# addam/mesh-reconstruction

Hardware: AMD Instinct MI355X
Metric: cost-volume samples/sec (pixels x planes x views) (higher is better)
Workload: dtype u8

## Files before the change

mesh-reconstruction_amd/csrc/sweep_rect.hip:

```cpp
#include "sweep_shared.hpp"

#include <cstddef>
#include <cstdio>
#include <cstdlib>
#include <cstring>
#include <type_traits>
#include <vector>

namespace mvs {

namespace {

constexpr float RX_MAGIC = 12582912.0f;
constexpr int RX_TILE_H = 8, RX_PC = 16, RX_KW = 4;
constexpr int RX_MAX_NI = 3;
#ifndef RX_DOUBLE_BUFFER
#define RX_DOUBLE_BUFFER 0
#endif
#ifndef RX_WAVES
#define RX_WAVES 5
#endif
constexpr int RX_WAVES_PER_SIMD = RX_WAVES;

enum RxMode : unsigned { RX_SKIP = 0, RX_FAST = 1, RX_BORDER = 2, RX_GENERIC = 3 };
// ... 247 lines not shown
    const RectCold *__restrict__ cold;
    uint2 *__restrict__ part;
    size_t pad_slab;
    int pitch, W, H, D, V, v0, vcount, nchunks, chunk0, chunk1, cps, ty0, tyn, tiles_x;
    int slot_dw;
};

template <typename T>
__device__ __forceinline__ T cold_get(uintptr_t c, size_t off)
{
    return *(const __attribute__((address_space(4))) T *)(c + off);
}
#define RX_COLD(c, T, field) cold_get<T>((uintptr_t)(c), offsetof(RectCold, field))

__device__ __forceinline__ __amdgpu_buffer_rsrc_t make_rsrc(const void *p, uint32_t bytes)
{
    return __builtin_amdgcn_make_buffer_rsrc((void *)p, 0, (int)bytes, 0x00020000);
}

template <int RS, bool WRITE_VOLUME, bool FUSED>
__global__ __launch_bounds__(256, RX_WAVES_PER_SIMD) void sweep_fx_rect(RectArgs a)
{
    constexpr int UNITS = RS / 4;
    constexpr int SLOT_BIAS_DW = RX_BIAS_X + RX_BIAS_Y * RS;
    extern __shared__ __attribute__((aligned(16))) uint32_t smem[];
    const uint32_t lds_base = (uint32_t)(size_t)(__attribute__((address_space(3))) void *)smem;

    const int band_tile = grouped_tile(blockIdx.x, a.tiles_x, a.tyn);
    if (band_tile < 0) return;
    const int tx = band_tile % a.tiles_x, ty = band_tile / a.tiles_x + a.ty0;
    const int lane = threadIdx.x & 63;
    const int wave = __builtin_amdgcn_readfirstlane((int)(threadIdx.x >> 6));
    const int col = tx * TILE_W + lane;
    const int row0 = ty * RX_TILE_H;
    const bool col_ok = col < a.W;
    const int NC = a.nchunks;

    uint32_t Im255[8];
    {
        const uint8_t *img = RX_COLD(a.cold, const uint8_t *, main_img);
#pragma unroll
        for (int j = 0; j < 8; j++) Im255[j] = (col_ok && row0 + j < a.H) ? 255u * (uint32_t)img[(size_t)(row0 + j) * a.W + col] : 0u;
    }

    uint32_t srcoff[RX_MAX_NI];
#pragma unroll
    for (int t = 0; t < RX_MAX_NI; t++) {
        const int g = (wave + 4 * t) * 64 + lane;
        srcoff[t] = 4u * (uint32_t)((g / UNITS) * a.pitch + (g % UNITS) * 4);
    }

    const int chunk_first = a.chunk0 + (int)blockIdx.y * a.cps;
    const int chunk_last = min(a.chunk1, chunk_first + a.cps);
    const int vend = a.v0 + a.vcount;
    const int nreg = (chunk_last - chunk_first) * a.vcount;

    const __amdgpu_buffer_rsrc_t rtab = make_rsrc(a.xw, 0xffffffffu);
    const uint32_t xw_wg = (uint32_t)(((size_t)tx * a.V * NC * 4 + wave) * 32);
    const uint32_t yr_wg = (uint32_t)((size_t)((const char *)a.yr - (const char *)a.xw) + ((size_t)ty * a.V * NC * 4 + wave) * 32);
    const __amdgpu_buffer_rsrc_t rquads = make_rsrc(a.quads, 0xffffffffu);

    auto issue_copy = [&](uint32_t xsx, uint32_t ysrc, uint32_t yn, uint32_t slot_dw0) {
        const int n = (int)((yn & 0xffu) * (xsx >> 16));
        const uint32_t src = (xsx & 0xffffu) + ysrc;
        uint32_t *dst = smem + slot_dw0 + SLOT_BIAS_DW + wave * 256;
        const int left = n - wave * 64;
        auto copy = [&](int t, bool whole) {
            int lim = left - 256 * t;
            asm volatile("" : "+s"(lim));
            if (whole || lane < lim)
                __builtin_amdgcn_raw_ptr_buffer_load_lds(rquads, (__attribute__((address_space(3))) void *)(dst + t * 1024), 16, srcoff[t], src, 0, 0);
        };
        static_assert(RX_MAX_NI == 3, "the nest below");
        if (left >= 64) {
            copy(0, true);
            if (left >= 320) {
                copy(1, true);
                if (left >= 576)
                    copy(2, true);
                else if (left > 512)
                    copy(2, false);
            } else if (left > 256) {
                copy(1, false);
            }
        } else if (left > 0) {
            copy(0, false);
        }
    };

    const uint32_t lane8 = 4u * (uint32_t)(lane & 7);
    auto load_x = [&](uint32_t xo) { return __builtin_amdgcn_raw_buffer_load_b32(rtab, lane8, xo, 0); };
    auto load_y = [&](uint32_t yo) { return __builtin_amdgcn_raw_buffer_load_b32(rtab, lane8, yo, 0); };
    auto rdl = [](uint32_t x, int l) { return (uint32_t)__builtin_amdgcn_readlane((int)x, l); };
    struct Cursor {
        int vleft, left;
        uint32_t xo;
    };
    const uint32_t xstep = 128u * (uint32_t)NC;
    const int vlast = a.vcount - 1;
    const uint32_t xwrap = 128u - xstep * (uint32_t)vlast;
    auto advance = [&](Cursor &c) {
        if (c.left <= 0) return;
        c.left--;
        const bool wrap = c.vleft == 0;
        c.xo += wrap ? xwrap : xstep;
        c.vleft = wrap ? vlast : c.vleft - 1;
    };
    const uint32_t x_first = xw_wg + 128u * (uint32_t)(a.v0 * NC + chunk_first);
    const uint32_t ydelta = yr_wg - xw_wg;

    uint32_t acc[8][RX_KW];
    uint32_t best[8];
    int bi[8];
#pragma unroll
    for (int j = 0; j < 8; j++) {
        best[j] = 0xffffffffu;
        bi[j] = -1;
#pragma unroll
        for (int k = 0; k < RX_KW; k++) acc[j][k] = 0u;
    }
    bool plain = true;
    uint32_t spacc = 0u;

    Cursor c2;
    c2.vleft = vlast;
    c2.left = nreg - 1;
    c2.xo = x_first;
    uint32_t x0r = load_x(c2.xo), y0r = load_y(c2.xo + ydelta);
    advance(c2);
    uint32_t x1r = load_x(c2.xo), y1r = load_y(c2.xo + ydelta);
    advance(c2);
    uint32_t slot_cur = 0u, slot_nxt = (uint32_t)a.slot_dw;
    if (nreg > 0) issue_copy(rdl(x0r, 6), rdl(y0r, 2), rdl(y0r, 3), slot_cur);
    int chunk = chunk_first, v = a.v0;

    for (int r = 0; r < nreg; r++) {
        wait_vm<0>();
        __builtin_amdgcn_s_barrier();
        if (r + 1 < nreg) issue_copy(rdl(x1r, 6), rdl(y1r, 2), rdl(y1r, 3), slot_nxt);
        const uint32_t x2r = load_x(c2.xo), y2r = load_y(c2.xo + ydelta);
        advance(c2);
        const uint32_t rsum = x0r + y0r;
        const uint32_t sum01 = rdl(rsum, 0), sum23 = rdl(rsum, 1);
        const uint32_t we[RX_KW] = {rdl(x0r, 2), rdl(x0r, 3), rdl(x0r, 4), rdl(x0r, 5)};
        const uint32_t fmask = 0xffffu;
        const uint32_t fld[RX_KW] = {sum01 & fmask, (sum01 >> 16) & fmask, sum23 & fmask, (sum23 >> 16) & fmask};

        const uint32_t special = (sum01 | sum23) & 0xc000c000u;
        {
            const uint32_t slot_byte = lds_base + slot_cur * 4u;
            uint32_t qd[1][8];
            const uint32_t xmasks = rdl(x0r, 7), ymasks = rdl(y0r, 4);
            const uint32_t anymask = xmasks | ymasks;
            if (__builtin_expect(anymask != 0u, 0)) {
#pragma unroll
                for (int k = 0; k < RX_KW; k++)
                    if (((anymask >> (8 * k)) & 0xffu) && !(fld[k] & 0xc000u)) spacc += 1u << (8 * k);
            }
#define RX_ROW_TAIL(j)                                                                                                   \
    "s_bitcmp0_b32 %[ym], %[yb" #j "]\n\ts_cselect_b64 exec, vcc, 0\n\tv_add_u32 %[a" #j "], 0x1000000, %[a" #j "]\n\t" \
    "v_sad_u16 %[a" #j "], %[q" #j "], %[i" #j "], %[a" #j "]\n\t"
#pragma unroll
            for (int k = 0; k < RX_KW; k++) {
#pragma clang diagnostic push
#pragma clang diagnostic ignored "-Winline-asm"
                asm volatile("s_add_u32 m0, %[slot], %[fld]\n\t"
                             "s_and_b32 vcc_lo, %[fld], 0xc000\n\t"
                             "ds_read_addtid_b32 %[q0] offset:%[o0]\n\tds_read_addtid_b32 %[q1] offset:%[o1]\n\tds_read_addtid_b32 %[q2] offset:%[o2]\n\tds_read_addtid_b32 %[q3] offset:%[o3]\n\t"
                             "ds_read_addtid_b32 %[q4] offset:%[o4]\n\tds_read_addtid_b32 %[q5] offset:%[o5]\n\tds_read_addtid_b32 %[q6] offset:%[o6]\n\tds_read_addtid_b32 %[q7] offset:%[o7]\n\t"
                             "s_cselect_b64 exec, 0, -1\n\t"
                             "s_bfe_u32 vcc_lo, %[am], %[kb]\n\t"
                             "s_cbranch_scc1 1f\n\t"
                             "s_waitcnt lgkmcnt(0)\n\t"
                             "v_dot4_u32_u8 %[q0], %[q0], %[w], 0\n\tv_dot4_u32_u8 %[q1], %[q1], %[w], 0\n\tv_dot4_u32_u8 %[q2], %[q2], %[w], 0\n\tv_dot4_u32_u8 %[q3], %[q3], %[w], 0\n\t"
                             "v_dot4_u32_u8 %[q4], %[q4], %[w], 0\n\tv_dot4_u32_u8 %[q5], %[q5], %[w], 0\n\tv_dot4_u32_u8 %[q6], %[q6], %[w], 0\n\tv_dot4_u32_u8 %[q7], %[q7], %[w], 0\n\t"
                             "v_sad_u16 %[a0], %[q0], %[i0], %[a0]\n\tv_sad_u16 %[a1], %[q1], %[i1], %[a1]\n\tv_sad_u16 %[a2], %[q2], %[i2], %[a2]\n\tv_sad_u16 %[a3], %[q3], %[i3], %[a3]\n\t"
                             "v_sad_u16 %[a4], %[q4], %[i4], %[a4]\n\tv_sad_u16 %[a5], %[q5], %[i5], %[a5]\n\tv_sad_u16 %[a6], %[q6], %[i6], %[a6]\n\tv_sad_u16 %[a7], %[q7], %[i7], %[a7]\n\t"
                             "2:\n\t"
                             "s_mov_b64 exec, -1\n\t"
                             "s_branch 9f\n\t"
                             "1:\n\t"
                             "s_bfe_u32 vcc_lo, %[xm], %[nb]\n\t"
                             "s_bitcmp1_b32 %[xm], %[sb]\n\t"
                             "s_cbranch_scc1 3f\n\t"
                             "s_lshl_b64 exec, exec, vcc_lo\n\t"
                             "s_branch 4f\n\t"
                             "3:\n\t"
                             "s_lshr_b64 exec, exec, vcc_lo\n\t"
                             "4:\n\t"
                             "s_bitcmp1_b32 %[xm], %[eb]\n\t"
                             "s_cselect_b64 exec, 0, exec\n\t"
                             "s_mov_b64 vcc, exec\n\t"
                             "s_waitcnt lgkmcnt(0)\n\t"
                             "v_dot4_u32_u8 %[q0], %[q0], %[w], 0\n\tv_dot4_u32_u8 %[q1], %[q1], %[w], 0\n\tv_dot4_u32_u8 %[q2], %[q2], %[w], 0\n\tv_dot4_u32_u8 %[q3], %[q3], %[w], 0\n\t"
                             "v_dot4_u32_u8 %[q4], %[q4], %[w], 0\n\tv_dot4_u32_u8 %[q5], %[q5], %[w], 0\n\tv_dot4_u32_u8 %[q6], %[q6], %[w], 0\n\tv_dot4_u32_u8 %[q7], %[q7], %[w], 0\n\t"
                             RX_ROW_TAIL(0) RX_ROW_TAIL(1) RX_ROW_TAIL(2) RX_ROW_TAIL(3) RX_ROW_TAIL(4) RX_ROW_TAIL(5) RX_ROW_TAIL(6) RX_ROW_TAIL(7)
                             "s_branch 2b\n\t"
                             "9:"
                             : [q0] "=&v"(qd[0][0]), [q1] "=&v"(qd[0][1]), [q2] "=&v"(qd[0][2]), [q3] "=&v"(qd[0][3]), [q4] "=&v"(qd[0][4]), [q5] "=&v"(qd[0][5]), [q6] "=&v"(qd[0][6]), [q7] "=&v"(qd[0][7]),
                               [a0] "+v"(acc[0][k]), [a1] "+v"(acc[1][k]), [a2] "+v"(acc[2][k]), [a3] "+v"(acc[3][k]), [a4] "+v"(acc[4][k]), [a5] "+v"(acc[5][k]), [a6] "+v"(acc[6][k]), [a7] "+v"(acc[7][k])
                             : [slot] "s"(slot_byte), [fld] "s"(fld[k]), [w] "s"(we[k]), [am] "s"(anymask), [xm] "s"(xmasks), [ym] "s"(ymasks),
                               [i0] "v"(Im255[0]), [i1] "v"(Im255[1]), [i2] "v"(Im255[2]), [i3] "v"(Im255[3]), [i4] "v"(Im255[4]), [i5] "v"(Im255[5]), [i6] "v"(Im255[6]), [i7] "v"(Im255[7]),
                               [o0] "n"(0), [o1] "n"(RS * 4), [o2] "n"(RS * 8), [o3] "n"(RS * 12), [o4] "n"(RS * 16), [o5] "n"(RS * 20), [o6] "n"(RS * 24), [o7] "n"(RS * 28),
                               [kb] "n"(8 * k | (8 << 16)), [nb] "n"(8 * k | (6 << 16)), [sb] "n"(8 * k + 7), [eb] "n"(8 * k + 6),
                               [yb0] "n"(8 * k + 0), [yb1] "n"(8 * k + 1), [yb2] "n"(8 * k + 2), [yb3] "n"(8 * k + 3), [yb4] "n"(8 * k + 4), [yb5] "n"(8 * k + 5), [yb6] "n"(8 * k + 6), [yb7] "n"(8 * k + 7)
                             : "m0", "scc", "vcc");
#pragma clang diagnostic pop
            }
#undef RX_ROW_TAIL
            if (special) {
                uintptr_t coldp = (uintptr_t)a.cold;
                asm volatile("" : "+s"(coldp));
                const int dpad = RX_COLD(coldp, int, dpad);
                const cu32 xt = as_const<cu32>(RX_COLD(coldp, const uint32_t *, xt) + ((size_t)tx * a.V + v) * dpad + chunk * RX_PC + wave * RX_KW);
                const cu32 yt = as_const<cu32>(RX_COLD(coldp, const uint32_t *, yt) + ((size_t)ty * a.V + v) * dpad + chunk * RX_PC + wave * RX_KW);
                const uint32_t xsx = rdl(x0r, 6), yn = rdl(y0r, 3);
                const int x0 = (int)((xsx & 0xffffu) >> 2), y0 = (int)((yn >> 8) & 0x3fffu);
                const bool staged = (xsx >> 16) != 0u && (yn & 0xffu) != 0u;
#pragma unroll
                for (int k = 0; k < RX_KW; k++) {
                    if (!(fld[k] & 0xc000u)) continue;
                    spacc += 1u << (8 * k);
                    if (!staged) continue;
                    const uint32_t xe = xt[k], ye = yt[k];
                    const int nx = (int)((xe >> 20) & 127u), ny = (int)((ye >> 20) & 127u);
                    if ((xe & ye) & RX_UNIFORM) {
                        if (nx >= TILE_W || ny >= RX_TILE_H) continue;
                        const int tx0 = (int)(xe & 0xfffffu) - RX_BIAS, ty0 = (int)(ye & 0xfffffu) - RX_BIAS;
                        const uint32_t addr = 4u * (uint32_t)lane + slot_byte + 4u * (uint32_t)(SLOT_BIAS_DW + ((ty0 >> 5) - y0) * RS + ((tx0 >> 5) - x0));
                        const bool lane_in = ((xe >> 27) & 1u) ? lane < TILE_W - nx : lane >= nx;
                        const int jlo = ((ye >> 27) & 1u) ? 0 : ny, jhi = ((ye >> 27) & 1u) ? RX_TILE_H - ny : RX_TILE_H;
                        if (lane_in) {
#pragma unroll
                            for (int j = 0; j < 8; j++) asm volatile("ds_read_b32 %0, %1 offset:%2" : "=v"(qd[0][j]) : "v"(addr), "n"(j * RS * 4));
                            asm volatile("s_waitcnt lgkmcnt(0)" : "+v"(qd[0][0]), "+v"(qd[0][1]), "+v"(qd[0][2]), "+v"(qd[0][3]), "+v"(qd[0][4]), "+v"(qd[0][5]), "+v"(qd[0][6]), "+v"(qd[0][7]));
#pragma unroll
                            for (int j = 0; j < 8; j++)
                                if (j >= jlo && j < jhi) acc[j][k] = sad_u16(__builtin_amdgcn_udot4(qd[0][j], we[k], 0u, false), Im255[j], acc[j][k] + (1u << 24));
                        }
                        continue;
                    }
                    const cf32 q = as_const<cf32>(RX_COLD(coldp, const float *, Q) + 12 * v);
                    const float z = as_const<cf32>(RX_COLD(coldp, const float *, z))[min(chunk * RX_PC + wave * RX_KW + k, a.D - 1)];
                    const float invW = RX_COLD(coldp, float, invW), invH = RX_COLD(coldp, float, invH);
                    const cu32 lut = as_const<cu32>(RX_COLD(coldp, const uint32_t *, lut));
                    const uint32_t lo_bits = __builtin_bit_cast(uint32_t, RX_MAGIC + 132.0f);
                    const uint32_t hix_bits = lo_bits + 256u * (uint32_t)a.W, hiy_bits = lo_bits + 256u * (uint32_t)a.H;
                    const float r256 = rect_r256(q);
                    const uint32_t txb = __builtin_bit_cast(uint32_t, rect_tx(q, r256, z, col, invW));
                    const bool inx = col_ok && txb > lo_bits && txb < hix_bits;
                    const int tx3 = (int)((txb & 0x3fffffu) >> 3) - 32 * lane;
                    const uint32_t tyv = __builtin_bit_cast(uint32_t, rect_ty(q, r256, z, row0 + (lane & 7), invH));
                    unsigned long long remaining = __builtin_amdgcn_ballot_w64(inx);
                    while (remaining) {
                        const int t = __builtin_amdgcn_readlane(tx3, (int)__builtin_ctzll(remaining));
                        const bool mine = inx && tx3 == t;
                        remaining &= ~__builtin_amdgcn_ballot_w64(mine);
                        const uint32_t kx = (uint32_t)t & 31u;
                        const int ixrel = (t >> 5) - x0;
#pragma unroll
                        for (int j = 0; j < 8; j++) {
                            const uint32_t tyb = (uint32_t)__builtin_amdgcn_readlane((int)tyv, j);
                            if (tyb > lo_bits && tyb < hiy_bits && row0 + j < a.H) {
                                const uint32_t uy = tyb & 0x3fffffu;
                                const uint32_t w = lut[((uy >> 3) & 31u) * 32u + kx];
                                const uint32_t addr = 4u * (uint32_t)lane + slot_byte + 4u * (uint32_t)(SLOT_BIAS_DW + ((int)(uy >> 8) - y0) * RS + ixrel);
                                if (mine) {
                                    uint32_t quad;
                                    asm volatile("ds_read_b32 %0, %1\n\ts_waitcnt lgkmcnt(0)" : "=v"(quad) : "v"(addr));
                                    acc[j][k] = sad_u16(__builtin_amdgcn_udot4(quad, w, 0u, false), Im255[j], acc[j][k] + (1u << 24));
                                }
                            }
                        }
                    }
                }
            }
        }

        if (v + 1 == vend) {
            const int d0 = chunk * RX_PC + wave * RX_KW;
            const size_t P = (size_t)a.W * a.H;
            const uint32_t pix0 = 4u * (uint32_t)(row0 * a.W + col);
            const int nrows = min(8, a.H - row0);
            if (FUSED && plain && spacc != 0u) {
                plain = false;
#pragma unroll
                for (int j = 0; j < 8; j++) best[j] = bi[j] < 0 ? 1u : best[j];
            }
            auto finish = [&](auto checked_rows, auto plain_compare) {
#pragma unroll
                for (int k = 0; k < RX_KW; k++) {
                    const uint32_t cntk = ((uint32_t)a.vcount - ((spacc >> (8 * k)) & 0xffu)) << 24;
                    if (d0 + k < a.D) {
                        const __amdgpu_buffer_rsrc_t rvol = make_rsrc(WRITE_VOLUME ? a.volume + (size_t)(d0 + k) * P : nullptr, 0xffffffffu);
#pragma unroll
                        for (int j = 0; j < 8; j++) {
                            if (!checked_rows.value || j < nrows) {
                                const uint32_t cell = acc[j][k] + cntk;
                                if (WRITE_VOLUME) __builtin_amdgcn_raw_buffer_store_b32(cell, rvol, pix0, 4u * (uint32_t)(j * a.W), 2);
                                if (FUSED) {
                                    const bool better = plain_compare.value ? cell < best[j] : umul24u(cell & 0xffffffu, best[j] >> 24) < umul24u(best[j] & 0xffffffu, cell >> 24);
                                    best[j] = better ? cell : best[j];
                                    bi[j] = better ? d0 + k : bi[j];
                                }
                            }
                        }
                    }
                }
            };
            if (col_ok) {
                if (nrows == 8 && plain)
                    finish(std::false_type{}, std::true_type{});
                else if (nrows == 8)
                    finish(std::false_type{}, std::false_type{});
                else if (plain)
                    finish(std::true_type{}, std::true_type{});
                else
                    finish(std::true_type{}, std::false_type{});
            }
#pragma unroll
            for (int k = 0; k < RX_KW; k++)
#pragma unroll
                for (int j = 0; j < 8; j++) acc[j][k] = 0u;
            spacc = 0u;
        }

        if (++v == vend) {
            v = a.v0;
            chunk++;
        }
        x0r = x1r;
        y0r = y1r;
        x1r = x2r;
        y1r = y2r;
        const uint32_t sw = slot_cur;
        slot_cur = slot_nxt;
        slot_nxt = sw;
    }

    if (FUSED) {
        __syncthreads();
        uint2 *ex = (uint2 *)smem;
#pragma unroll
        for (int j = 0; j < 8; j++) ex[(wave * 8 + j) * 64 + lane] = make_uint2(best[j], (uint32_t)bi[j]);
        __syncthreads();
        const size_t P = (size_t)a.W * a.H;
        float *depth = RX_COLD(a.cold, float *, depth), *cost = RX_COLD(a.cold, float *, cost);
        int *index = RX_COLD(a.cold, int *, index);
        const float *zt = RX_COLD(a.cold, const float *, z);
#pragma unroll
        for (int jj = 0; jj < 2; jj++) {
            const int j = wave * 2 + jj;
            const int row = row0 + j;
            if (col_ok && row < a.H) {
                uint32_t b = 1u;
                int bidx = -1;
#pragma unroll
                for (int s = 0; s < 4; s++) {
                    const uint2 c = ex[(s * 8 + j) * 64 + lane];
                    if ((int)c.y >= 0) {
                        const uint32_t lhs = umul24u(c.x & 0xffffffu, b >> 24), rhs = umul24u(b & 0xffffffu, c.x >> 24);
                        const bool take = lhs < rhs || (lhs == rhs && bidx >= 0 && (int)c.y < bidx);
                        b = take ? c.x : b;
                        bidx = take ? (int)c.y : bidx;
                    }
                }
                if (bidx < 0) b = 0u;
                const size_t pix = (size_t)row * a.W + col;
                if (a.part) {
                    a.part[(size_t)blockIdx.y * P + pix] = make_uint2(b, (uint32_t)bidx);
                } else {
                    depth[pix] = bidx >= 0 ? zt[bidx] : MVS_BACKGROUND_DEPTH;
                    cost[pix] = bidx >= 0 ? cell_cost<CS_FIXED>(b & 0xffffffu, b >> 24) : __builtin_inff();
                    index[pix] = bidx;
                }
            }
        }
    }
}

int ensure_fx_lut(mvs_ctx *ctx);

bool rect_view_host(const float *q) { return q[1] == 0.0f && q[4] == 0.0f && q[8] == 0.0f && q[9] == 0.0f && q[10] == 0.0f && q[11] > 0.0f; }

struct RectSizes {
    size_t nx, ny, nw, nxw, nyr, nxb, nyb, total;
};

static RectSizes rect_sizes(const SweepParams &q)
{
    RectSizes z;
    const size_t dpad = (size_t)q.nchunks * RX_PC;
    z.nx = (size_t)q.tiles_x * q.V * dpad;
    z.ny = (size_t)q.tiles_y * q.V * dpad;
    z.nw = (size_t)q.V * dpad;
    z.nxb = (size_t)q.tiles_x * q.V * q.nchunks;
    z.nyb = (size_t)q.tiles_y * q.V * q.nchunks;
    z.nxw = z.nxb * 32;
    z.nyr = z.nyb * 32;
    z.total = 16 + z.nxw + z.nyr + 2 * z.nx + 2 * z.ny + z.nw + z.nxb + z.nyb + 64;
    return z;
}

static void rect_tables(mvs_ctx *ctx, const SweepParams &q, RectTables &rt)
{
    const RectSizes z = rect_sizes(q);
    uint32_t *base = (uint32_t *)ctx->rect_tab.ptr;
    rt.dpad = q.nchunks * RX_PC;
    rt.stats = (int *)base;
    rt.xw = base + 16;
    rt.yr = rt.xw + z.nxw;
    rt.xt = rt.yr + z.nyr;
    rt.yt = rt.xt + z.nx;
    rt.wt = rt.yt + z.ny;
    rt.xmm = rt.wt + z.nw;
    rt.ymm = rt.xmm + z.nx;
    rt.xbox = rt.ymm + z.ny;
    rt.ybox = rt.xbox + z.nxb;
}

static size_t rect_table_dwords(const SweepParams &q) { return rect_sizes(q).total; }

int sweep_rect_plan(mvs_ctx *ctx, PlanHook *between)
{
    struct RunHookOnce {
        PlanHook *h;
        int rc = MVS_OK;
        bool done = false;
        int go()
        {
            if (!done && h) rc = h->run();
            done = true;
            return rc;
        }
    } hook{between};
    ctx->rect_ok = false;
    ctx->rect_cold_sent = false;
    if (ctx->hooks.no_rect) return hook.go();
    if (ctx->V == 0) return hook.go();
    for (int v = 0; v < ctx->V; v++)
        if (!rect_view_host(ctx->q_host.data() + 12 * v)) return hook.go();
    if ((unsigned long long)ctx->pad_slab * (unsigned long long)(ctx->views_in_store ? ctx->store_cap : ctx->V) * 4ull >= (1ull << 32)) return hook.go();
    SweepParams q;
    fill_params(ctx, q, 0, ctx->V, RX_TILE_H, RX_PC);
    int rc;
    if ((rc = ensure(ctx, ctx->rect_tab, rect_table_dwords(q) * sizeof(uint32_t) + sizeof(RectCold) + 256)) || (rc = ensure_fx_lut(ctx))) {
        (void)hook.go();
        return rc;
    }
    if (!ctx->plan_event) MVS_HIP(ctx, hipEventCreateWithFlags(&ctx->plan_event, hipEventDisableTiming));
    RectTables rt;
    rect_tables(ctx, q, rt);
    MVS_HIP(ctx, hipMemsetAsync(rt.stats, 0, 64, ctx->stream));
    const size_t na = (size_t)(q.tiles_x + q.tiles_y + 1) * q.V * rt.dpad;
    plan_rect_axis<<<(unsigned)((na + 255) / 256), 256, 0, ctx->stream>>>(q, rt, (const uint32_t *)ctx->fx_lut.ptr);
    const size_t nb = (size_t)(q.tiles_x + q.tiles_y) * q.V * q.nchunks;
    plan_rect_box<<<(unsigned)((nb + 255) / 256), 256, 0, ctx->stream>>>(q, rt);
    MVS_HIP(ctx, hipGetLastError());
    int stats[4] = {0, 0, 0, 0};
    MVS_HIP(ctx, hipMemcpyAsync(stats, rt.stats, sizeof(stats), hipMemcpyDeviceToHost, ctx->stream));
    MVS_HIP(ctx, hipEventRecord(ctx->plan_event, ctx->stream));
    if ((rc = hook.go())) return rc;
    MVS_HIP(ctx, hipEventSynchronize(ctx->plan_event));
    const int max_rw = stats[0], max_rh = stats[1];
    int rs = 0;
    if (ctx->hooks.rect_verbose) fprintf(stderr, "sweep_rect_plan: widest box %d quads, tallest %d rows\n", max_rw, max_rh);
    for (int cand : {64, 84, 96, 128})
        if (max_rw <= cand) {
            rs = cand;
            break;
        }
    if (!rs || max_rw <= 0 || max_rh <= 0 || max_rh > 32) return MVS_OK;
    const int units = rs / 4;
    const int instrs = div_up(max_rh * units, 64);
    if (instrs > 4 * RX_MAX_NI || instrs * 1024 >= 16384) return MVS_OK;
    if (4 * (rs + RX_BIAS_X) + 4 * rs * (max_rh + RX_BIAS_Y) >= 16384) return MVS_OK;
    ctx->rect_rs = rs;
    ctx->rect_slot_dw = instrs * 256;
    ctx->rect_dpad = rt.dpad;
    plan_rect_pack<<<(unsigned)((4 * nb + 255) / 256), 256, 0, ctx->stream>>>(q, rt, rs);
    MVS_HIP(ctx, hipGetLastError());
    RectCold cold;
    cold.main_img = main_image_ptr(ctx);
    cold.xt = rt.xt;
    cold.yt = rt.yt;
    cold.lut = (const uint32_t *)ctx->fx_lut.ptr;
    cold.Q = (const float *)ctx->qmats.ptr;
    cold.z = (const float *)ctx->ztab.ptr;
    cold.depth = (float *)ctx->depth.ptr;
    cold.cost = (float *)ctx->cost.ptr;
    cold.index = (int *)ctx->index.ptr;
    cold.invW = q.invW;
    cold.invH = q.invH;
    cold.dpad = rt.dpad;
    cold.pad_ = 0;
    ctx->rect_cold_host.resize(sizeof(RectCold));
    memcpy(ctx->rect_cold_host.data(), &cold, sizeof(RectCold));
    ctx->rect_ok = true;
    return MVS_OK;
}

template <int RS>
static int launch_rect(mvs_ctx *ctx, const RectArgs &a, dim3 grid, size_t lds, bool vol, bool fused)
{
    auto go = [&](auto kernel) -> int {
        MVS_HIP(ctx, hipFuncSetAttribute((const void *)kernel, hipFuncAttributeMaxDynamicSharedMemorySize, (int)lds));
        kernel<<<grid, 256, lds, ctx->stream>>>(a);
        MVS_HIP(ctx, hipGetLastError());
        return MVS_OK;
    };
    if (vol && fused) return go(sweep_fx_rect<RS, true, true>);
    if (vol) return go(sweep_fx_rect<RS, true, false>);
    return go(sweep_fx_rect<RS, false, true>);
}

int sweep_rect_launch(mvs_ctx *ctx, SweepParams &p, bool vol, bool fused, unsigned flags)
{
    RectTables rt;
    rect_tables(ctx, p, rt);
    RectCold *cold_dev = (RectCold *)((uint32_t *)ctx->rect_tab.ptr + rect_table_dwords(p));
    RectCold cold;
    memcpy(&cold, ctx->rect_cold_host.data(), sizeof(RectCold));
    cold.main_img = main_image_ptr(ctx);
    cold.depth = (float *)ctx->depth.ptr;
    cold.cost = (float *)ctx->cost.ptr;
    cold.index = (int *)ctx->index.ptr;
    if (!ctx->rect_cold_sent || memcmp(&cold, ctx->rect_cold_host.data(), sizeof(RectCold)) != 0) {
        memcpy(ctx->rect_cold_host.data(), &cold, sizeof(RectCold));
        MVS_HIP(ctx, hipMemcpyAsync(cold_dev, ctx->rect_cold_host.data(), sizeof(RectCold), hipMemcpyHostToDevice, ctx->stream));
        ctx->rect_cold_sent = true;
    }
    RectArgs a;
    a.quads = p.quads;
    a.xw = rt.xw;
    a.yr = rt.yr;
    a.volume = p.volume;
    a.cold = cold_dev;
    a.part = nullptr;
    a.pad_slab = p.pad_slab;
    a.pitch = p.pitch;
    a.W = p.W;
    a.H = p.H;
    a.D = p.D;
    a.V = p.V;
    a.v0 = p.v0;
    a.vcount = p.vcount;
    a.nchunks = p.nchunks;
    a.chunk0 = p.chunk0;
    a.chunk1 = p.chunk1;
    a.ty0 = p.ty0;
    a.tyn = p.tyn;
    a.tiles_x = p.tiles_x;
    a.slot_dw = ctx->rect_slot_dw;
    size_t lds = ((size_t)2 * a.slot_dw + RX_BIAS_X + (size_t)RX_BIAS_Y * ctx->rect_rs) * 4;
    if (fused) lds = lds < 16384 ? 16384 : lds;
    if (lds > 160 * 1024) return fail(ctx, MVS_EINVAL, "sweep_rect_launch: %zu bytes of LDS", lds);

    const int groups = div_up(p.tiles_x, 2) * div_up(p.tyn, 4);
    const int nch = p.chunk1 - p.chunk0, tiles = p.tiles_x * p.tyn;
    int want = (int)((flags >> 16) & 0xffu);
    if (!want) want = div_up(16 * ctx->num_cus, tiles);
    p.cps = div_up(nch, max(1, min(want, nch)));
    a.cps = p.cps;
    const int nsplit = div_up(nch, p.cps);
    int rc;
    if (fused && nsplit > 1) {
        if ((rc = ensure(ctx, ctx->best_parts, (size_t)nsplit * ctx->W * ctx->H * sizeof(uint2)))) return rc;
        p.part = (uint2 *)ctx->best_parts.ptr;
        a.part = p.part;
    }
    const dim3 grid((unsigned)(div_up(groups, 8) * 64), (unsigned)nsplit);
    rc = ctx->rect_rs == 64 ? launch_rect<64>(ctx, a, grid, lds, vol, fused) : ctx->rect_rs == 84 ? launch_rect<84>(ctx, a, grid, lds, vol, fused)
       : ctx->rect_rs == 96 ? launch_rect<96>(ctx, a, grid, lds, vol, fused) : launch_rect<128>(ctx, a, grid, lds, vol, fused);
    if (rc) return rc;
    return nsplit;
}

}
```

Measured before the change: 6999 billion.

## Add fused four-plane fast path with software-pipelined LDS reads for clean regions

When a region has no special, masked or border planes, one asm block now processes all four planes. LDS reads for the next plane are interleaved with the SAD ops of the current one, and staggered lgkmcnt waits replace the full wait per plane. Regions that are not clean fall back to the old per-plane masked path, which now also skips planes that are fully out of frame. A verbose-only host diagnostic reports the fraction of clean regions. The cost is more live VGPRs from holding all four accumulator sets and the weights in one asm block, which could lower occupancy.

```diff
diff --git a/mesh-reconstruction_amd/csrc/sweep_rect.hip b/mesh-reconstruction_amd/csrc/sweep_rect.hip
--- a/mesh-reconstruction_amd/csrc/sweep_rect.hip
+++ b/mesh-reconstruction_amd/csrc/sweep_rect.hip
@@ -423,123 +423,168 @@
             uint32_t qd[1][8];
             const uint32_t xmasks = rdl(x0r, 7), ymasks = rdl(y0r, 4);
             const uint32_t anymask = xmasks | ymasks;
-            if (__builtin_expect(anymask != 0u, 0)) {
-#pragma unroll
-                for (int k = 0; k < RX_KW; k++)
-                    if (((anymask >> (8 * k)) & 0xffu) && !(fld[k] & 0xc000u)) spacc += 1u << (8 * k);
-            }
-#define RX_ROW_TAIL(j)                                                                                                   \
-    "s_bitcmp0_b32 %[ym], %[yb" #j "]\n\ts_cselect_b64 exec, vcc, 0\n\tv_add_u32 %[a" #j "], 0x1000000, %[a" #j "]\n\t" \
-    "v_sad_u16 %[a" #j "], %[q" #j "], %[i" #j "], %[a" #j "]\n\t"
-#pragma unroll
-            for (int k = 0; k < RX_KW; k++) {
+            const uint32_t clean = special | anymask;
+            {
+#define RX_RD(j) "ds_read_addtid_b32 %[q" #j "] offset:%[o" #j "]\n\t"
+#define RX_DOT(j, k) "v_dot4_u32_u8 %[q" #j "], %[q" #j "], %[w" #k "], 0\n\t"
+#define RX_SAD(j, k) "v_sad_u16 %[a" #j #k "], %[q" #j "], %[i" #j "], %[a" #j #k "]\n\t"
+#define RX_DOTS(k)                                                                                                        \
+    "s_waitcnt lgkmcnt(6)\n\t" RX_DOT(0, k) RX_DOT(1, k) "s_waitcnt lgkmcnt(4)\n\t" RX_DOT(2, k) RX_DOT(3, k)                \
+    "s_waitcnt lgkmcnt(2)\n\t" RX_DOT(4, k) RX_DOT(5, k) "s_waitcnt lgkmcnt(0)\n\t" RX_DOT(6, k) RX_DOT(7, k)
+#define RX_PLANE(k, kn)                                                                                                   \
+    RX_DOTS(k) "s_add_u32 m0, %[slot], %[f" #kn "]\n\t"                                                                  \
+    RX_SAD(0, k) RX_RD(0) RX_SAD(1, k) RX_RD(1) RX_SAD(2, k) RX_RD(2) RX_SAD(3, k) RX_RD(3)                                  \
+    RX_SAD(4, k) RX_RD(4) RX_SAD(5, k) RX_RD(5) RX_SAD(6, k) RX_RD(6) RX_SAD(7, k) RX_RD(7)
+#define RX_ACC(k)                                                                                                         \
+    [a0##k] "+v"(acc[0][k]), [a1##k] "+v"(acc[1][k]), [a2##k] "+v"(acc[2][k]), [a3##k] "+v"(acc[3][k]),                   \
+    [a4##k] "+v"(acc[4][k]), [a5##k] "+v"(acc[5][k]), [a6##k] "+v"(acc[6][k]), [a7##k] "+v"(acc[7][k])
 #pragma clang diagnostic push
 #pragma clang diagnostic ignored "-Winline-asm"
-                asm volatile("s_add_u32 m0, %[slot], %[fld]\n\t"
-                             "s_and_b32 vcc_lo, %[fld], 0xc000\n\t"
-                             "ds_read_addtid_b32 %[q0] offset:%[o0]\n\tds_read_addtid_b32 %[q1] offset:%[o1]\n\tds_read_addtid_b32 %[q2] offset:%[o2]\n\tds_read_addtid_b32 %[q3] offset:%[o3]\n\t"
-                             "ds_read_addtid_b32 %[q4] offset:%[o4]\n\tds_read_addtid_b32 %[q5] offset:%[o5]\n\tds_read_addtid_b32 %[q6] offset:%[o6]\n\tds_read_addtid_b32 %[q7] offset:%[o7]\n\t"
-                             "s_cselect_b64 exec, 0, -1\n\t"
-                             "s_bfe_u32 vcc_lo, %[am], %[kb]\n\t"
-                             "s_cbranch_scc1 1f\n\t"
+                asm volatile("s_cmp_lg_u32 %[cl], 0\n\t"
+                             "s_cbranch_scc1 9f\n\t"
                              "s_waitcnt lgkmcnt(0)\n\t"
-                             "v_dot4_u32_u8 %[q0], %[q0], %[w], 0\n\tv_dot4_u32_u8 %[q1], %[q1], %[w], 0\n\tv_dot4_u32_u8 %[q2], %[q2], %[w], 0\n\tv_dot4_u32_u8 %[q3], %[q3], %[w], 0\n\t"
-                             "v_dot4_u32_u8 %[q4], %[q4], %[w], 0\n\tv_dot4_u32_u8 %[q5], %[q5], %[w], 0\n\tv_dot4_u32_u8 %[q6], %[q6], %[w], 0\n\tv_dot4_u32_u8 %[q7], %[q7], %[w], 0\n\t"
-                             "v_sad_u16 %[a0], %[q0], %[i0], %[a0]\n\tv_sad_u16 %[a1], %[q1], %[i1], %[a1]\n\tv_sad_u16 %[a2], %[q2], %[i2], %[a2]\n\tv_sad_u16 %[a3], %[q3], %[i3], %[a3]\n\t"
-                             "v_sad_u16 %[a4], %[q4], %[i4], %[a4]\n\tv_sad_u16 %[a5], %[q5], %[i5], %[a5]\n\tv_sad_u16 %[a6], %[q6], %[i6], %[a6]\n\tv_sad_u16 %[a7], %[q7], %[i7], %[a7]\n\t"
-                             "2:\n\t"
-                             "s_mov_b64 exec, -1\n\t"
-                             "s_branch 9f\n\t"
-                             "1:\n\t"
-                             "s_bfe_u32 vcc_lo, %[xm], %[nb]\n\t"
-                             "s_bitcmp1_b32 %[xm], %[sb]\n\t"
-                             "s_cbranch_scc1 3f\n\t"
-                             "s_lshl_b64 exec, exec, vcc_lo\n\t"
-                             "s_branch 4f\n\t"
-                             "3:\n\t"
-                             "s_lshr_b64 exec, exec, vcc_lo\n\t"
-                             "4:\n\t"
-                             "s_bitcmp1_b32 %[xm], %[eb]\n\t"
-                             "s_cselect_b64 exec, 0, exec\n\t"
-                             "s_mov_b64 vcc, exec\n\t"
-                             "s_waitcnt lgkmcnt(0)\n\t"
-                             "v_dot4_u32_u8 %[q0], %[q0], %[w], 0\n\tv_dot4_u32_u8 %[q1], %[q1], %[w], 0\n\tv_dot4_u32_u8 %[q2], %[q2], %[w], 0\n\tv_dot4_u32_u8 %[q3], %[q3], %[w], 0\n\t"
-                             "v_dot4_u32_u8 %[q4], %[q4], %[w], 0\n\tv_dot4_u32_u8 %[q5], %[q5], %[w], 0\n\tv_dot4_u32_u8 %[q6], %[q6], %[w], 0\n\tv_dot4_u32_u8 %[q7], %[q7], %[w], 0\n\t"
-                             RX_ROW_TAIL(0) RX_ROW_TAIL(1) RX_ROW_TAIL(2) RX_ROW_TAIL(3) RX_ROW_TAIL(4) RX_ROW_TAIL(5) RX_ROW_TAIL(6) RX_ROW_TAIL(7)
-                             "s_branch 2b\n\t"
+                             "s_add_u32 m0, %[slot], %[f0]\n\t"
+                             "s_nop 0\n\t"
+                             RX_RD(0) RX_RD(1) RX_RD(2) RX_RD(3) RX_RD(4) RX_RD(5) RX_RD(6) RX_RD(7)
+                             RX_PLANE(0, 1) RX_PLANE(1, 2) RX_PLANE(2, 3)
+                             RX_DOTS(3)
+                             RX_SAD(0, 3) RX_SAD(1, 3) RX_SAD(2, 3) RX_SAD(3, 3) RX_SAD(4, 3) RX_SAD(5, 3) RX_SAD(6, 3) RX_SAD(7, 3)
                              "9:"
                              : [q0] "=&v"(qd[0][0]), [q1] "=&v"(qd[0][1]), [q2] "=&v"(qd[0][2]), [q3] "=&v"(qd[0][3]), [q4] "=&v"(qd[0][4]), [q5] "=&v"(qd[0][5]), [q6] "=&v"(qd[0][6]), [q7] "=&v"(qd[0][7]),
-                               [a0] "+v"(acc[0][k]), [a1] "+v"(acc[1][k]), [a2] "+v"(acc[2][k]), [a3] "+v"(acc[3][k]), [a4] "+v"(acc[4][k]), [a5] "+v"(acc[5][k]), [a6] "+v"(acc[6][k]), [a7] "+v"(acc[7][k])
-                             : [slot] "s"(slot_byte), [fld] "s"(fld[k]), [w] "s"(we[k]), [am] "s"(anymask), [xm] "s"(xmasks), [ym] "s"(ymasks),
+                               RX_ACC(0), RX_ACC(1), RX_ACC(2), RX_ACC(3)
+                             : [cl] "s"(clean), [slot] "s"(slot_byte), [f0] "s"(fld[0]), [f1] "s"(fld[1]), [f2] "s"(fld[2]), [f3] "s"(fld[3]),
+                               [w0] "s"(we[0]), [w1] "s"(we[1]), [w2] "s"(we[2]), [w3] "s"(we[3]),
                                [i0] "v"(Im255[0]), [i1] "v"(Im255[1]), [i2] "v"(Im255[2]), [i3] "v"(Im255[3]), [i4] "v"(Im255[4]), [i5] "v"(Im255[5]), [i6] "v"(Im255[6]), [i7] "v"(Im255[7]),
-                               [o0] "n"(0), [o1] "n"(RS * 4), [o2] "n"(RS * 8), [o3] "n"(RS * 12), [o4] "n"(RS * 16), [o5] "n"(RS * 20), [o6] "n"(RS * 24), [o7] "n"(RS * 28),
-                               [kb] "n"(8 * k | (8 << 16)), [nb] "n"(8 * k | (6 << 16)), [sb] "n"(8 * k + 7), [eb] "n"(8 * k + 6),
-                               [yb0] "n"(8 * k + 0), [yb1] "n"(8 * k + 1), [yb2] "n"(8 * k + 2), [yb3] "n"(8 * k + 3), [yb4] "n"(8 * k + 4), [yb5] "n"(8 * k + 5), [yb6] "n"(8 * k + 6), [yb7] "n"(8 * k + 7)
-                             : "m0", "scc", "vcc");
+                               [o0] "n"(0), [o1] "n"(RS * 4), [o2] "n"(RS * 8), [o3] "n"(RS * 12), [o4] "n"(RS * 16), [o5] "n"(RS * 20), [o6] "n"(RS * 24), [o7] "n"(RS * 28)
+                             : "m0", "scc");
 #pragma clang diagnostic pop
+#undef RX_ACC
+#undef RX_PLANE
+#undef RX_DOTS
+#undef RX_SAD
+#undef RX_DOT
+#undef RX_RD
             }
+            if (__builtin_expect(clean != 0u, 0)) {
+                if (__builtin_expect(anymask != 0u, 0)) {
+#pragma unroll
+                    for (int k = 0; k < RX_KW; k++)
+                        if (((anymask >> (8 * k)) & 0xffu) && !(fld[k] & 0xc000u)) spacc += 1u << (8 * k);
+                }
+#define RX_ROW_TAIL(j)                                                                                                   \
+        "s_bitcmp0_b32 %[ym], %[yb" #j "]\n\ts_cselect_b64 exec, vcc, 0\n\tv_add_u32 %[a" #j "], 0x1000000, %[a" #j "]\n\t" \
+        "v_sad_u16 %[a" #j "], %[q" #j "], %[i" #j "], %[a" #j "]\n\t"
+#pragma unroll
+                for (int k = 0; k < RX_KW; k++) {
+                    if ((((xmasks >> (8 * k)) & 0x40u) | (((ymasks >> (8 * k)) & 0xffu) == 0xffu)) != 0u) continue;
+#pragma clang diagnostic push
+#pragma clang diagnostic ignored "-Winline-asm"
+                    asm volatile("s_add_u32 m0, %[slot], %[fld]\n\t"
+                                 "s_and_b32 vcc_lo, %[fld], 0xc000\n\t"
+                                 "ds_read_addtid_b32 %[q0] offset:%[o0]\n\tds_read_addtid_b32 %[q1] offset:%[o1]\n\tds_read_addtid_b32 %[q2] offset:%[o2]\n\tds_read_addtid_b32 %[q3] offset:%[o3]\n\t"
+                                 "ds_read_addtid_b32 %[q4] offset:%[o4]\n\tds_read_addtid_b32 %[q5] offset:%[o5]\n\tds_read_addtid_b32 %[q6] offset:%[o6]\n\tds_read_addtid_b32 %[q7] offset:%[o7]\n\t"
+                                 "s_cselect_b64 exec, 0, -1\n\t"
+                                 "s_bfe_u32 vcc_lo, %[am], %[kb]\n\t"
+                                 "s_cbranch_scc1 1f\n\t"
+                                 "s_waitcnt lgkmcnt(0)\n\t"
+                                 "v_dot4_u32_u8 %[q0], %[q0], %[w], 0\n\tv_dot4_u32_u8 %[q1], %[q1], %[w], 0\n\tv_dot4_u32_u8 %[q2], %[q2], %[w], 0\n\tv_dot4_u32_u8 %[q3], %[q3], %[w], 0\n\t"
+                                 "v_dot4_u32_u8 %[q4], %[q4], %[w], 0\n\tv_dot4_u32_u8 %[q5], %[q5], %[w], 0\n\tv_dot4_u32_u8 %[q6], %[q6], %[w], 0\n\tv_dot4_u32_u8 %[q7], %[q7], %[w], 0\n\t"
+                                 "v_sad_u16 %[a0], %[q0], %[i0], %[a0]\n\tv_sad_u16 %[a1], %[q1], %[i1], %[a1]\n\tv_sad_u16 %[a2], %[q2], %[i2], %[a2]\n\tv_sad_u16 %[a3], %[q3], %[i3], %[a3]\n\t"
+                                 "v_sad_u16 %[a4], %[q4], %[i4], %[a4]\n\tv_sad_u16 %[a5], %[q5], %[i5], %[a5]\n\tv_sad_u16 %[a6], %[q6], %[i6], %[a6]\n\tv_sad_u16 %[a7], %[q7], %[i7], %[a7]\n\t"
+                                 "2:\n\t"
+                                 "s_mov_b64 exec, -1\n\t"
+                                 "s_branch 9f\n\t"
+                                 "1:\n\t"
+                                 "s_bfe_u32 vcc_lo, %[xm], %[nb]\n\t"
+                                 "s_bitcmp1_b32 %[xm], %[sb]\n\t"
+                                 "s_cbranch_scc1 3f\n\t"
+                                 "s_lshl_b64 exec, exec, vcc_lo\n\t"
+                                 "s_branch 4f\n\t"
+                                 "3:\n\t"
+                                 "s_lshr_b64 exec, exec, vcc_lo\n\t"
+                                 "4:\n\t"
+                                 "s_bitcmp1_b32 %[xm], %[eb]\n\t"
+                                 "s_cselect_b64 exec, 0, exec\n\t"
+                                 "s_mov_b64 vcc, exec\n\t"
+                                 "s_waitcnt lgkmcnt(0)\n\t"
+                                 "v_dot4_u32_u8 %[q0], %[q0], %[w], 0\n\tv_dot4_u32_u8 %[q1], %[q1], %[w], 0\n\tv_dot4_u32_u8 %[q2], %[q2], %[w], 0\n\tv_dot4_u32_u8 %[q3], %[q3], %[w], 0\n\t"
+                                 "v_dot4_u32_u8 %[q4], %[q4], %[w], 0\n\tv_dot4_u32_u8 %[q5], %[q5], %[w], 0\n\tv_dot4_u32_u8 %[q6], %[q6], %[w], 0\n\tv_dot4_u32_u8 %[q7], %[q7], %[w], 0\n\t"
+                                 RX_ROW_TAIL(0) RX_ROW_TAIL(1) RX_ROW_TAIL(2) RX_ROW_TAIL(3) RX_ROW_TAIL(4) RX_ROW_TAIL(5) RX_ROW_TAIL(6) RX_ROW_TAIL(7)
+                                 "s_branch 2b\n\t"
+                                 "9:"
+                                 : [q0] "=&v"(qd[0][0]), [q1] "=&v"(qd[0][1]), [q2] "=&v"(qd[0][2]), [q3] "=&v"(qd[0][3]), [q4] "=&v"(qd[0][4]), [q5] "=&v"(qd[0][5]), [q6] "=&v"(qd[0][6]), [q7] "=&v"(qd[0][7]),
+                                   [a0] "+v"(acc[0][k]), [a1] "+v"(acc[1][k]), [a2] "+v"(acc[2][k]), [a3] "+v"(acc[3][k]), [a4] "+v"(acc[4][k]), [a5] "+v"(acc[5][k]), [a6] "+v"(acc[6][k]), [a7] "+v"(acc[7][k])
+                                 : [slot] "s"(slot_byte), [fld] "s"(fld[k]), [w] "s"(we[k]), [am] "s"(anymask), [xm] "s"(xmasks), [ym] "s"(ymasks),
+                                   [i0] "v"(Im255[0]), [i1] "v"(Im255[1]), [i2] "v"(Im255[2]), [i3] "v"(Im255[3]), [i4] "v"(Im255[4]), [i5] "v"(Im255[5]), [i6] "v"(Im255[6]), [i7] "v"(Im255[7]),
+                                   [o0] "n"(0), [o1] "n"(RS * 4), [o2] "n"(RS * 8), [o3] "n"(RS * 12), [o4] "n"(RS * 16), [o5] "n"(RS * 20), [o6] "n"(RS * 24), [o7] "n"(RS * 28),
+                                   [kb] "n"(8 * k | (8 << 16)), [nb] "n"(8 * k | (6 << 16)), [sb] "n"(8 * k + 7), [eb] "n"(8 * k + 6),
+                                   [yb0] "n"(8 * k + 0), [yb1] "n"(8 * k + 1), [yb2] "n"(8 * k + 2), [yb3] "n"(8 * k + 3), [yb4] "n"(8 * k + 4), [yb5] "n"(8 * k + 5), [yb6] "n"(8 * k + 6), [yb7] "n"(8 * k + 7)
+                                 : "m0", "scc", "vcc");
+#pragma clang diagnostic pop
+                }
 #undef RX_ROW_TAIL
-            if (special) {
-                uintptr_t coldp = (uintptr_t)a.cold;
-                asm volatile("" : "+s"(coldp));
-                const int dpad = RX_COLD(coldp, int, dpad);
-                const cu32 xt = as_const<cu32>(RX_COLD(coldp, const uint32_t *, xt) + ((size_t)tx * a.V + v) * dpad + chunk * RX_PC + wave * RX_KW);
-                const cu32 yt = as_const<cu32>(RX_COLD(coldp, const uint32_t *, yt) + ((size_t)ty * a.V + v) * dpad + chunk * RX_PC + wave * RX_KW);
-                const uint32_t xsx = rdl(x0r, 6), yn = rdl(y0r, 3);
-                const int x0 = (int)((xsx & 0xffffu) >> 2), y0 = (int)((yn >> 8) & 0x3fffu);
-                const bool staged = (xsx >> 16) != 0u && (yn & 0xffu) != 0u;
-#pragma unroll
-                for (int k = 0; k < RX_KW; k++) {
-                    if (!(fld[k] & 0xc000u)) continue;
-                    spacc += 1u << (8 * k);
-                    if (!staged) continue;
-                    const uint32_t xe = xt[k], ye = yt[k];
-                    const int nx = (int)((xe >> 20) & 127u), ny = (int)((ye >> 20) & 127u);
-                    if ((xe & ye) & RX_UNIFORM) {
-                        if (nx >= TILE_W || ny >= RX_TILE_H) continue;
-                        const int tx0 = (int)(xe & 0xfffffu) - RX_BIAS, ty0 = (int)(ye & 0xfffffu) - RX_BIAS;
-                        const uint32_t addr = 4u * (uint32_t)lane + slot_byte + 4u * (uint32_t)(SLOT_BIAS_DW + ((ty0 >> 5) - y0) * RS + ((tx0 >> 5) - x0));
-                        const bool lane_in = ((xe >> 27) & 1u) ? lane < TILE_W - nx : lane >= nx;
-                        const int jlo = ((ye >> 27) & 1u) ? 0 : ny, jhi = ((ye >> 27) & 1u) ? RX_TILE_H - ny : RX_TILE_H;
-                        if (lane_in) {
-#pragma unroll
-                            for (int j = 0; j < 8; j++) asm volatile("ds_read_b32 %0, %1 offset:%2" : "=v"(qd[0][j]) : "v"(addr), "n"(j * RS * 4));
-                            asm volatile("s_waitcnt lgkmcnt(0)" : "+v"(qd[0][0]), "+v"(qd[0][1]), "+v"(qd[0][2]), "+v"(qd[0][3]), "+v"(qd[0][4]), "+v"(qd[0][5]), "+v"(qd[0][6]), "+v"(qd[0][7]));
-#pragma unroll
-                            for (int j = 0; j < 8; j++)
-                                if (j >= jlo && j < jhi) acc[j][k] = sad_u16(__builtin_amdgcn_udot4(qd[0][j], we[k], 0u, false), Im255[j], acc[j][k] + (1u << 24));
+                if (special) {
+                    uintptr_t coldp = (uintptr_t)a.cold;
+                    asm volatile("" : "+s"(coldp));
+                    const int dpad = RX_COLD(coldp, int, dpad);
+                    const cu32 xt = as_const<cu32>(RX_COLD(coldp, const uint32_t *, xt) + ((size_t)tx * a.V + v) * dpad + chunk * RX_PC + wave * RX_KW);
+                    const cu32 yt = as_const<cu32>(RX_COLD(coldp, const uint32_t *, yt) + ((size_t)ty * a.V + v) * dpad + chunk * RX_PC + wave * RX_KW);
+                    const uint32_t xsx = rdl(x0r, 6), yn = rdl(y0r, 3);
+                    const int x0 = (int)((xsx & 0xffffu) >> 2), y0 = (int)((yn >> 8) & 0x3fffu);
+                    const bool staged = (xsx >> 16) != 0u && (yn & 0xffu) != 0u;
+#pragma unroll
+                    for (int k = 0; k < RX_KW; k++) {
+                        if (!(fld[k] & 0xc000u)) continue;
+                        spacc += 1u << (8 * k);
+                        if (!staged) continue;
+                        const uint32_t xe = xt[k], ye = yt[k];
+                        const int nx = (int)((xe >> 20) & 127u), ny = (int)((ye >> 20) & 127u);
+                        if ((xe & ye) & RX_UNIFORM) {
+                            if (nx >= TILE_W || ny >= RX_TILE_H) continue;
+                            const int tx0 = (int)(xe & 0xfffffu) - RX_BIAS, ty0 = (int)(ye & 0xfffffu) - RX_BIAS;
+                            const uint32_t addr = 4u * (uint32_t)lane + slot_byte + 4u * (uint32_t)(SLOT_BIAS_DW + ((ty0 >> 5) - y0) * RS + ((tx0 >> 5) - x0));
+                            const bool lane_in = ((xe >> 27) & 1u) ? lane < TILE_W - nx : lane >= nx;
+                            const int jlo = ((ye >> 27) & 1u) ? 0 : ny, jhi = ((ye >> 27) & 1u) ? RX_TILE_H - ny : RX_TILE_H;
+                            if (lane_in) {
+#pragma unroll
+                                for (int j = 0; j < 8; j++) asm volatile("ds_read_b32 %0, %1 offset:%2" : "=v"(qd[0][j]) : "v"(addr), "n"(j * RS * 4));
+                                asm volatile("s_waitcnt lgkmcnt(0)" : "+v"(qd[0][0]), "+v"(qd[0][1]), "+v"(qd[0][2]), "+v"(qd[0][3]), "+v"(qd[0][4]), "+v"(qd[0][5]), "+v"(qd[0][6]), "+v"(qd[0][7]));
+#pragma unroll
+                                for (int j = 0; j < 8; j++)
+                                    if (j >= jlo && j < jhi) acc[j][k] = sad_u16(__builtin_amdgcn_udot4(qd[0][j], we[k], 0u, false), Im255[j], acc[j][k] + (1u << 24));
+                            }
+                            continue;
                         }
-                        continue;
-                    }
-                    const cf32 q = as_const<cf32>(RX_COLD(coldp, const float *, Q) + 12 * v);
-                    const float z = as_const<cf32>(RX_COLD(coldp, const float *, z))[min(chunk * RX_PC + wave * RX_KW + k, a.D - 1)];
-                    const float invW = RX_COLD(coldp, float, invW), invH = RX_COLD(coldp, float, invH);
-                    const cu32 lut = as_const<cu32>(RX_COLD(coldp, const uint32_t *, lut));
-                    const uint32_t lo_bits = __builtin_bit_cast(uint32_t, RX_MAGIC + 132.0f);
-                    const uint32_t hix_bits = lo_bits + 256u * (uint32_t)a.W, hiy_bits = lo_bits + 256u * (uint32_t)a.H;
-                    const float r256 = rect_r256(q);
-                    const uint32_t txb = __builtin_bit_cast(uint32_t, rect_tx(q, r256, z, col, invW));
-                    const bool inx = col_ok && txb > lo_bits && txb < hix_bits;
-                    const int tx3 = (int)((txb & 0x3fffffu) >> 3) - 32 * lane;
-                    const uint32_t tyv = __builtin_bit_cast(uint32_t, rect_ty(q, r256, z, row0 + (lane & 7), invH));
-                    unsigned long long remaining = __builtin_amdgcn_ballot_w64(inx);
-                    while (remaining) {
-                        const int t = __builtin_amdgcn_readlane(tx3, (int)__builtin_ctzll(remaining));
-                        const bool mine = inx && tx3 == t;
-                        remaining &= ~__builtin_amdgcn_ballot_w64(mine);
-                        const uint32_t kx = (uint32_t)t & 31u;
-                        const int ixrel = (t >> 5) - x0;
-#pragma unroll
-                        for (int j = 0; j < 8; j++) {
-                            const uint32_t tyb = (uint32_t)__builtin_amdgcn_readlane((int)tyv, j);
-                            if (tyb > lo_bits && tyb < hiy_bits && row0 + j < a.H) {
-                                const uint32_t uy = tyb & 0x3fffffu;
-                                const uint32_t w = lut[((uy >> 3) & 31u) * 32u + kx];
-                                const uint32_t addr = 4u * (uint32_t)lane + slot_byte + 4u * (uint32_t)(SLOT_BIAS_DW + ((int)(uy >> 8) - y0) * RS + ixrel);
-                                if (mine) {
-                                    uint32_t quad;
-                                    asm volatile("ds_read_b32 %0, %1\n\ts_waitcnt lgkmcnt(0)" : "=v"(quad) : "v"(addr));
-                                    acc[j][k] = sad_u16(__builtin_amdgcn_udot4(quad, w, 0u, false), Im255[j], acc[j][k] + (1u << 24));
+                        const cf32 q = as_const<cf32>(RX_COLD(coldp, const float *, Q) + 12 * v);
+                        const float z = as_const<cf32>(RX_COLD(coldp, const float *, z))[min(chunk * RX_PC + wave * RX_KW + k, a.D - 1)];
+                        const float invW = RX_COLD(coldp, float, invW), invH = RX_COLD(coldp, float, invH);
+                        const cu32 lut = as_const<cu32>(RX_COLD(coldp, const uint32_t *, lut));
+                        const uint32_t lo_bits = __builtin_bit_cast(uint32_t, RX_MAGIC + 132.0f);
+                        const uint32_t hix_bits = lo_bits + 256u * (uint32_t)a.W, hiy_bits = lo_bits + 256u * (uint32_t)a.H;
+                        const float r256 = rect_r256(q);
+                        const uint32_t txb = __builtin_bit_cast(uint32_t, rect_tx(q, r256, z, col, invW));
+                        const bool inx = col_ok && txb > lo_bits && txb < hix_bits;
+                        const int tx3 = (int)((txb & 0x3fffffu) >> 3) - 32 * lane;
+                        const uint32_t tyv = __builtin_bit_cast(uint32_t, rect_ty(q, r256, z, row0 + (lane & 7), invH));
+                        unsigned long long remaining = __builtin_amdgcn_ballot_w64(inx);
+                        while (remaining) {
+                            const int t = __builtin_amdgcn_readlane(tx3, (int)__builtin_ctzll(remaining));
+                            const bool mine = inx && tx3 == t;
+                            remaining &= ~__builtin_amdgcn_ballot_w64(mine);
+                            const uint32_t kx = (uint32_t)t & 31u;
+                            const int ixrel = (t >> 5) - x0;
+#pragma unroll
+                            for (int j = 0; j < 8; j++) {
+                                const uint32_t tyb = (uint32_t)__builtin_amdgcn_readlane((int)tyv, j);
+                                if (tyb > lo_bits && tyb < hiy_bits && row0 + j < a.H) {
+                                    const uint32_t uy = tyb & 0x3fffffu;
+                                    const uint32_t w = lut[((uy >> 3) & 31u) * 32u + kx];
+                                    const uint32_t addr = 4u * (uint32_t)lane + slot_byte + 4u * (uint32_t)(SLOT_BIAS_DW + ((int)(uy >> 8) - y0) * RS + ixrel);
+                                    if (mine) {
+                                        uint32_t quad;
+                                        asm volatile("ds_read_b32 %0, %1\n\ts_waitcnt lgkmcnt(0)" : "=v"(quad) : "v"(addr));
+                                        acc[j][k] = sad_u16(__builtin_amdgcn_udot4(quad, w, 0u, false), Im255[j], acc[j][k] + (1u << 24));
+                                    }
                                 }
                             }
                         }
@@ -751,6 +796,57 @@
     ctx->rect_dpad = rt.dpad;
     plan_rect_pack<<<(unsigned)((4 * nb + 255) / 256), 256, 0, ctx->stream>>>(q, rt, rs);
     MVS_HIP(ctx, hipGetLastError());
+    if (ctx->hooks.rect_verbose) {
+        const RectSizes z = rect_sizes(q);
+        std::vector<uint32_t> xw(z.nxw), yr(z.nyr);
+        MVS_HIP(ctx, hipMemcpyAsync(xw.data(), rt.xw, z.nxw * 4, hipMemcpyDeviceToHost, ctx->stream));
+        MVS_HIP(ctx, hipMemcpyAsync(yr.data(), rt.yr, z.nyr * 4, hipMemcpyDeviceToHost, ctx->stream));
+        MVS_HIP(ctx, hipStreamSynchronize(ctx->stream));
+        const size_t per = (size_t)q.V * q.nchunks * 4;
+        const double TX = q.tiles_x, TY = q.tiles_y;
+        double clean = 0.0, none = 0.0, flagged = 0.0, side[4] = {0.0, 0.0, 0.0, 0.0};
+        for (size_t e = 0; e < per; e++) {
+            size_t cx = 0, cy = 0;
+            for (int t = 0; t < q.tiles_x; t++) {
+                const uint32_t *r = xw.data() + ((size_t)t * per + e) * 8;
+                cx += ((r[0] | r[1]) & 0x40004000u) == 0u && r[7] == 0u;
+            }
+            for (int t = 0; t < q.tiles_y; t++) {
+                const uint32_t *r = yr.data() + ((size_t)t * per + e) * 8;
+                cy += ((r[0] | r[1]) & 0x80008000u) == 0u && r[4] == 0u;
+            }
+            clean += (double)cx * (double)cy;
+            for (int k = 0; k < RX_KW; k++) {
+                double xn = 0, xf = 0, yn = 0, yf = 0, l = 0, rt_ = 0, tp = 0, bt = 0;
+                for (int t = 0; t < q.tiles_x; t++) {
+                    const uint32_t *r = xw.data() + ((size_t)t * per + e) * 8;
+                    const uint32_t f = (r[k >> 1] >> (16 * (k & 1))) & 0xffffu, m = (r[7] >> (8 * k)) & 0xffu;
+                    xf += (f & 0x4000u) != 0u;
+                    xn += (m & 0x40u) != 0u;
+                    l += m != 0u && !(m & 0x40u) && !(m & 0x80u);
+                    rt_ += m != 0u && !(m & 0x40u) && (m & 0x80u);
+                }
+                for (int t = 0; t < q.tiles_y; t++) {
+                    const uint32_t *r = yr.data() + ((size_t)t * per + e) * 8;
+                    const uint32_t f = (r[k >> 1] >> (16 * (k & 1))) & 0xffffu, m = (r[4] >> (8 * k)) & 0xffu;
+                    yf += (f & 0x8000u) != 0u;
+                    yn += m == 0xffu;
+                    tp += m != 0u && m != 0xffu && (m & 1u);
+                    bt += m != 0u && m != 0xffu && (m & 0x80u);
+                }
+                none += TX * TY - (TX - xn) * (TY - yn);
+                flagged += TX * TY - (TX - xf) * (TY - yf);
+                side[0] += l * TY;
+                side[1] += rt_ * TY;
+                side[2] += tp * TX;
+                side[3] += bt * TX;
+            }
+        }
+        const double nreg = (double)per * TX * TY, npl = nreg * RX_KW;
+        fprintf(stderr, "sweep_rect_plan: clean regions %.2f %% of %.0f; planes: nothing in frame %.3f %%, failed certificate %.3f %%, "
+                "border left %.3f %% right %.3f %% top %.3f %% bottom %.3f %%\n", 100.0 * clean / nreg, nreg, 100.0 * none / npl,
+                100.0 * flagged / npl, 100.0 * side[0] / npl, 100.0 * side[1] / npl, 100.0 * side[2] / npl, 100.0 * side[3] / npl);
+    }
     RectCold cold;
     cold.main_img = main_image_ptr(ctx);
     cold.xt = rt.xt;
```

After: 7707 billion, median of 6. 10.1% higher.
